# GEOS-ESM/QuickChem

Hardware: AMD Instinct MI355X
Metric: OH gridcells/sec (XGBoost predict), C360 L72 batch (higher is better)
Workload: dtype f32

## Files before the change

quickchem_amd/capi.py:

```python
from __future__ import annotations

import ctypes as C
import os
from typing import Optional, Sequence

import numpy as np

_HERE = os.path.dirname(os.path.abspath(__file__))
LIB_PATH = os.path.join(_HERE, "lib", "libohxgb.so")
RING_ROUNDS_DEFAULT = 64
RING_ROUNDS_NO_GRID = 16
RING_ROUNDS_PERMUTED = 4
VISITS_BLOCK_ROWS = 256
VISITS_LDS_BLOCKS_PER_CU = 1
VISITS_GLOBAL_BLOCKS_PER_CU = 4

ABI_SYMBOLS = [
    "XGBGetLastError", "XGDMatrixCreateFromMat", "XGDMatrixFree", "XGDMatrixNumRow", "XGDMatrixNumCol",
    "XGDMatrixSaveBinary", "XGDMatrixCreateFromFile", "XGBoosterCreate", "XGBoosterFree", "XGBoosterLoadModel",
    "XGBoosterSaveModel", "XGBoosterLoadModelFromBuffer", "XGBoosterPredict", "XGBoosterSetParam",
    "OHXDeviceCount", "OHXDMatrixCreateFromDevice", "OHXDMatrixSetGrid", "OHXDMatrixGetGrid", "OHXDMatrixInferGrid", "OHXBoosterPredictDevice", "OHXBoosterCheck",
    "OHXBoosterPredictContribs", "OHXBoosterPredictContribsDevice",
    "OHXBoosterPredictInteractions", "OHXBoosterPredictInteractionsDevice",
    "OHXBoosterPredictContribsFields", "OHXBoosterPredictContribsFieldsDevice",
    "OHXBoosterCountVisits", "OHXBoosterCountVisitsDevice", "OHXBoosterGetVisitCounts", "OHXBoosterResetVisitCounts",
    "OHXBoosterRefreshCover", "OHXBoosterRefitLeaves", "OHXBoosterRefitLeavesDevice",
    "OHXBoosterBoostTrees", "OHXBoosterBoostTreesDevice", "OHXBoosterBoostTreesEval", "OHXBoosterBoostTreesEvalDevice",
    "OHXBoosterBoostTreesWeighted", "OHXBoosterBoostTreesWeightedDevice",
    "OHXBoosterBoostTreesSampled", "OHXBoosterBoostTreesSampledDevice",
    "OHXBoosterBoostTreesDeep", "OHXBoosterBoostTreesDeepDevice",
    "OHXBoosterBoostTreesDeepSampled", "OHXBoosterBoostTreesDeepSampledDevice",
    "OHXQuantileCuts", "OHXDMatrixQuantileCuts",
    "OHXSelectCells", "OHXSelectCellsDevice", "OHXGatherCells", "OHXGatherCellsDevice",
    "OHXScatterCells", "OHXScatterCellsDevice",
    "OHXBoosterPredictFields", "OHXBoosterPredictFieldsDevice", "OHXBoosterRun1", "OHXBoosterRun1Device", "OHXOHPostProcess", "OHXOHPostProcessDevice",
    "OHXJulianDay", "OHXSolarGeometry", "OHXSolarGeometryDevice", "OHXBoosterGetInfo", "OHXBoosterGetNumGroups", "OHXBoosterGetNumCategoricalSplits", "OHXBoosterKernelSymbol", "OHXBoosterKernelSymbolRows",
    "OHXBoosterRingReruns", "OHXBoosterCopyEngineChoice", "OHXUnregisterHost", "OHXReleaseScratch",
    "OHXCommGetUniqueId", "OHXCommInitRank", "OHXCommFree", "OHXCommInfo", "OHXShardRows", "OHXAllGatherOH",
]
REFERENCE_BOUND_SYMBOLS = [
    "XGBoosterLoadModel", "XGBoosterSaveModel", "XGDMatrixSaveBinary", "XGDMatrixFree", "XGDMatrixCreateFromFile",
    "XGBoosterPredict", "XGBoosterCreate", "XGDMatrixCreateFromMat", "XGDMatrixNumRow", "XGDMatrixNumCol",
    "XGBoosterFree",
# ... 1008 lines not shown
```

quickchem_amd/csrc/capi.cpp:

```cpp
#include <hip/hip_runtime_api.h>

#include <algorithm>
#include <cmath>
#include <cstdio>
#include <cstdlib>
#include <cstring>
#include <fstream>
#include <map>
#include <memory>
#include <atomic>
#include <chrono>
#include <mutex>
#include <unordered_map>
#include <sstream>
#include <string>
#include <unordered_set>
#include <vector>

#include "../../include/ohxgb.h"
#include "categorical.hpp"
#include "cells.hpp"
#include "contribs.hpp"
#include "flatten.hpp"
#include "forest.hpp"
// ... 812 lines not shown
  b.dev = use_device(b.device_pref);
  const Forest& flat = b.flat();
  b.placement = place_forest(flat, b.layout);
  b.packed_ok = packed_format_fits(flat, b.placement);
  b.d_roots.upload(b.placement.roots);
  if (b.num_cat != 0) {
    CatForest cf = emit_cat(flat, b.placement);
    b.cat_word_count = cf.words.size();
    b.cat_inline_sets = cf.inline_sets;
    b.cat_word_sets = cf.word_sets;
    if (cf.words.empty()) cf.words.push_back(0u);
    b.d_cat_nodes.upload(cf.nodes);
    b.d_cat_words.upload(cf.words);
    b.d_cat_orig.upload(cf.orig_id);
  } else if (wants_super(b.kernel_name)) {
    SuperForest sf;
    b.super_ok = emit_super(flat, &sf, b.layout.super_pack) && sf.nodes.size() * sizeof(SuperNode) < 0xFFFFFFF0ull;
    if (b.super_ok) {
      b.super_slots = sf.nodes.size();
      b.super_gathers[0] = count_super_gathers(sf, 0);
      b.super_gathers[1] = count_super_gathers(sf, 1);
      b.super_gathers[2] = count_super_gathers(sf, 2);
      b.super_mean_steps = mean_super_steps(sf);
      b.d_super.upload(sf.nodes);
      if (((uintptr_t)b.d_super.p & 127u) != 0) throw OhxError("internal error: the super-node array is not 128-byte aligned");
      b.d_super_heads.upload(sf.heads);
    }
  }
  if (b.num_cat == 0 && b.packed_ok && !(b.super_ok && wants_super(b.kernel_name))) {
    std::vector<PackedNode> packed = emit_packed(flat, b.placement, nullptr);
    b.d_packed.upload(packed);
  }
  if (b.num_cat == 0 && pick_kernel(b) == KernelKind::Wide) ensure_wide(b);
  b.d_flags.ensure(3);
  {
    LibStreams& ls = lib_streams(b.dev.ordinal);
    b.s_exec = ls.exec;
    b.s_copy = ls.copy;
  }
  HIP_CHECK(hipMemsetAsync(b.d_flags.p, 0, 3 * sizeof(uint32_t), b.s_exec));
  HIP_CHECK(hipStreamSynchronize(b.s_exec));
  b.ring_reruns_seen = 0;
  ensure_train_stream(b);
  b.uploaded = true;
}

void ensure_train_stream(BoosterObj& b) {
  b.tune.train = nullptr;
  if (b.tune.overlap_group < 2) return;
  if (!b.train.side) {
    HIP_CHECK(hipStreamCreateWithFlags(&b.train.side, hipStreamNonBlocking));
    HIP_CHECK(hipEventCreateWithFlags(&b.train.fork, hipEventDisableTiming));
    HIP_CHECK(hipEventCreateWithFlags(&b.train.join, hipEventDisableTiming));
  }
  b.tune.train = &b.train;
}

DeviceForest device_forest(const BoosterObj& b) {
  DeviceForest d;
  d.packed = b.d_packed.p;
  d.wide = b.d_wide.p;
  d.roots = b.d_roots.p;
  d.super = b.d_super.p;
  d.super_heads = b.d_super_heads.p;
  d.packed_bytes = (uint32_t)(b.d_packed.n * sizeof(PackedNode));
  d.super_bytes = (uint32_t)(b.d_super.n * sizeof(SuperNode));
  d.num_trees = (uint32_t)b.forest.trees.size();
  d.num_feature = b.forest.num_feature;
  d.base_score = b.margin_base;
  d.tree_tops = (b.super_ok && use_tree_tops(b.tune, b.super_mean_steps)) ? 1u : 0u;
  return d;
}

// ... 3833 lines not shown
```

quickchem_amd/csrc/kernels.hip:

```cpp
#include <hip/hip_runtime.h>

#include <atomic>

#include <cstdint>

#include "kernels.hpp"
#include "walk_device.hpp"

namespace ohx {

namespace {

constexpr int kBlock = 256;
constexpr int kWavesPerBlock = kBlock / kWave;

typedef const __attribute__((address_space(3))) char* lds_cptr;
typedef const __attribute__((address_space(3))) u32x4* lds_u32x4_ptr;
typedef __attribute__((address_space(3))) uint32_t* lds_u32_ptr;
typedef __attribute__((address_space(3))) void* lds_void_ptr;


__device__ __forceinline__ uint64_t launch_row(const PredictArgs& a, uint64_t tile_id, int lane, bool* valid,
                                               uint64_t perm_slots = ~0ull) {
  if (a.perm != nullptr) {
// ... 624 lines not shown
        const bool lane_nan = stage_rows<true>(tile, a.rows, row, valid, a.ncol, fr.num_feature, a.missing,
                                               missing_is_nan, a.flags);
        float* leaves = a.leaf_buf + ((size_t)(tile_id - a.tile_begin) * ntree - a.tree_begin) * kWave + lane;
        (void)walk_tile<FMT, CHAINS, TOPS>(fr, heads, t0, t1, tile, __any(lane_nan), first, nfirst, leaves);
      }
      return;
    }
  }
  uint64_t slots = ~0ull, tile_end = a.tile_end;
  if (a.perm_count != nullptr) {
    const uint32_t filled = *a.perm_count;
    slots = filled < a.perm_slots ? filled : a.perm_slots;
    const uint64_t need = (slots + kWave - 1) / kWave;
    tile_end = need < tile_end ? need : tile_end;
  }
  for (uint64_t tile_id = a.tile_begin + wave_id; tile_id < tile_end; tile_id += nwaves) {
    bool valid;
    const uint64_t row = launch_row(a, tile_id, lane, &valid, slots);
    if (!__any(valid)) continue;
    const bool lane_nan = stage_rows<true>(tile, a.rows, row, valid, a.ncol, fr.num_feature, a.missing,
                                           missing_is_nan, a.flags);
    const bool wave_nan = __any(lane_nan);
    const float acc = walk_tile<FMT, CHAINS, TOPS>(fr, heads, a.tree_begin, a.tree_end, tile, wave_nan, first, nfirst);
    if (valid) __builtin_nontemporal_store(acc, out + row);
  }
}

constexpr int kRingChains = 4;
constexpr int kRingWaves = 16;
constexpr int kRingBlock = kRingWaves * kWave;
constexpr uint32_t kRingSteps = 4;
constexpr uint32_t kRingSlots = 176;
constexpr uint32_t kRingBuffers = 4;
constexpr uint32_t kRingTreeBytes = kRingSlots * 16u;
constexpr uint32_t kRingBufBytes = kRingChains * kRingTreeBytes;
constexpr uint32_t kRingDmaLoads = kRingChains * kRingSlots / kWave;
static_assert(kRingChains * kRingSlots % kWave == 0, "a group is whole wave loads");
#ifndef OHX_EXP_RING_SPIN
#define OHX_EXP_RING_SPIN (1u << 21)
#endif
constexpr uint32_t kRingSpinLimit = OHX_EXP_RING_SPIN;
constexpr size_t kRingLdsBytes = (size_t)kRingWaves * 27 * kWave * sizeof(float) + (size_t)kRingBuffers * kRingBufBytes +
                                 (size_t)(kRingWaves + 4) * sizeof(uint32_t);
static_assert(kRingLdsBytes <= 160 * 1024, "LDS of a block");

__device__ __forceinline__ uint32_t ring_load(lds_u32_ptr p) {
  return __hip_atomic_load(p, __ATOMIC_RELAXED, __HIP_MEMORY_SCOPE_WORKGROUP);
}
__device__ __forceinline__ void ring_store(lds_u32_ptr p, uint32_t v) {
  __hip_atomic_store(p, v, __ATOMIC_RELAXED, __HIP_MEMORY_SCOPE_WORKGROUP);
}
__device__ __forceinline__ void ring_order() { asm volatile("s_waitcnt lgkmcnt(0)" ::: "memory"); }

__device__ __forceinline__ void dma_to_lds_b128(u32x4 desc, uint32_t off, uint32_t lds_addr) {
#if defined(__gfx950__)
  uint32_t keep;
  const uint32_t m0_value = (uint32_t)__builtin_amdgcn_readfirstlane((int)lds_addr);
  asm volatile(
      "s_mov_b32 %0, m0\n\ts_mov_b32 m0, %3\n\ts_nop 0\n\tbuffer_load_dwordx4 %1, %2, 0 offen lds\n\ts_mov_b32 m0, %0"
      : "=&s"(keep)
      : "v"(off), "s"(desc), "s"(m0_value)
      : "memory");
#else
  (void)desc; (void)off; (void)lds_addr;
  __builtin_trap();
#endif
}

struct TopRing {
  lds_cptr ring;
  uint32_t ring_addr;
  lds_u32_ptr progress, filled, claim, abort;
  u32x4 desc;
  __amdgpu_buffer_rsrc_t forest;
  const SuperTreeHead* heads;
  uint32_t t0, t1, ngroups;
  uint32_t total;
  uint32_t g;
  bool gave_up;
};

__device__ __forceinline__ void ring_stage(const TopRing& rg, uint32_t first_tree, uint32_t buf, int lane) {
  uint32_t base[kRingChains];
#pragma unroll
  for (int c = 0; c < kRingChains; ++c) base[c] = rg.heads[(first_tree + c < rg.t1) ? first_tree + c : rg.t1 - 1].base;
#pragma unroll
  for (uint32_t q = 0; q < kRingDmaLoads; ++q) {
    const uint32_t L = q * kWave + (uint32_t)lane;
    uint32_t b = base[0], rec = L;
#pragma unroll
    for (int k = 1; k < kRingChains; ++k)
      if (L >= (uint32_t)k * kRingSlots) b = base[k], rec = L - (uint32_t)k * kRingSlots;
    dma_to_lds_b128(rg.desc, (b + rec) << 4, rg.ring_addr + buf * kRingBufBytes + q * 1024u);
  }
}

__device__ __forceinline__ void ring_begin(TopRing& rg, char* ring, const DeviceForest& fr, const SuperTreeHead* heads,
                                           uint32_t t0, uint32_t t1, uint32_t rounds) {
  const int lane = threadIdx.x & (kWave - 1);
  rg.ring = (lds_cptr)ring;
  rg.ring_addr = (uint32_t)(uintptr_t)(lds_void_ptr)ring;
  rg.progress = (lds_u32_ptr)(ring + (size_t)kRingBuffers * kRingBufBytes);
  rg.filled = rg.progress + kRingWaves;
  rg.claim = rg.progress + kRingWaves + 1;
  rg.abort = rg.progress + kRingWaves + 2;
  const uint64_t addr = reinterpret_cast<uint64_t>(fr.super);
  rg.desc.x = (uint32_t)__builtin_amdgcn_readfirstlane((int)(uint32_t)addr);
  rg.desc.y = (uint32_t)__builtin_amdgcn_readfirstlane((int)((uint32_t)(addr >> 32) & 0xFFFFu));
  rg.desc.z = (uint32_t)__builtin_amdgcn_readfirstlane((int)fr.super_bytes);
  rg.desc.w = 0x00020000u;
  rg.forest = make_rsrc(fr.super, fr.super_bytes);
  rg.heads = heads;
  rg.t0 = t0;
  rg.t1 = t1;
  rg.ngroups = (t1 - t0 + kRingChains - 1) / kRingChains;
  rg.total = rounds * rg.ngroups;
  rg.g = 0;
  rg.gave_up = false;
  if (threadIdx.x < kWave) {
    ring_stage(rg, t0, 0u, lane);
    asm volatile("s_waitcnt vmcnt(0)" ::: "memory");
  }
  if (threadIdx.x < (uint32_t)kRingWaves) ring_store(rg.progress + threadIdx.x, 0u);
  if (threadIdx.x == 0) {
    ring_store(rg.filled, 1u);
    ring_store(rg.claim, 1u);
    ring_store(rg.abort, 0u);
  }
  __syncthreads();
}

template <bool HAS_MISSING>
__device__ __forceinline__ float ring_walk_group(const SuperTreeHead (&h)[kRingChains], uint32_t ntrees_here,
                                                 __amdgpu_buffer_rsrc_t forest, const float* __restrict__ tile,
                                                 lds_cptr tops, float acc, lds_u32_ptr publish_to,
                                                 uint32_t publish_value, bool ahead) {
  constexpr int CHAINS = kRingChains;
  const char* tile_b = reinterpret_cast<const char*>(tile);
  __builtin_amdgcn_s_setprio(1);
  u32x4 s[CHAINS];
  uint32_t rel[CHAINS], leafb[CHAINS];
  float xr[CHAINS];
#pragma unroll
  for (int c = 0; c < CHAINS; ++c) xr[c] = tile[(h[c].root_meta & 31u) * kWave];
#pragma unroll
  for (int c = 0; c < CHAINS; ++c) {
    bool l = xr[c] < h[c].root_thr;
    if (HAS_MISSING) l = go_left_or_default(xr[c], h[c].root_thr, (h[c].root_meta & 32u) != 0u);
    rel[c] = 4u + (((h[c].root_meta & 0x100u) && !l) ? 1u : 0u);
    leafb[c] = 0u;
  }
  uint32_t nsteps = h[0].steps;
#pragma unroll
  for (int c = 1; c < CHAINS; ++c) nsteps = h[c].steps > nsteps ? h[c].steps : nsteps;
  nsteps = nsteps < kRingSteps ? kRingSteps : nsteps;
#pragma unroll
  for (int c = 0; c < CHAINS; ++c) s[c] = *(lds_u32x4_ptr)(tops + (uint32_t)c * kRingTreeBytes + (rel[c] << 4));
#pragma unroll
  for (uint32_t step = 1; step < kRingSteps; ++step) {
    if (step == 2 && !ahead) __builtin_amdgcn_s_setprio(2);
    super_step<CHAINS, HAS_MISSING, false>(s, rel, leafb, tile_b);
#pragma unroll
    for (int c = 0; c < CHAINS; ++c) s[c] = *(lds_u32x4_ptr)(tops + (uint32_t)c * kRingTreeBytes + (rel[c] << 4));
  }
  if (publish_to != nullptr) {
    asm volatile("s_waitcnt vmcnt(0)" ::: "memory");
    if ((threadIdx.x & (kWave - 1)) == 0) ring_store(publish_to, publish_value);
  }
  if (ahead) __builtin_amdgcn_s_setprio(2);
  else __builtin_amdgcn_s_setprio(3);
  uint32_t base[CHAINS];
#pragma unroll
  for (int c = 0; c < CHAINS; ++c) base[c] = h[c].base;
  for (uint32_t step = kRingSteps; step < nsteps; ++step)
    super_step_by_chain<CHAINS, HAS_MISSING>(s, rel, leafb, tile_b, [&](int c, uint32_t record) -> u32x4 {
      return __builtin_amdgcn_raw_buffer_load_b128(forest, (int)((base[c] + record) << 4), 0, 0);
    });
  super_step<CHAINS, HAS_MISSING, true>(s, rel, leafb, tile_b);
  __builtin_amdgcn_s_setprio(1);
#pragma unroll
  for (int c = 0; c < CHAINS; ++c)
    if ((uint32_t)c < ntrees_here) acc += __uint_as_float(leafb[c]);
  return acc;
}

__device__ __forceinline__ bool ring_aborted(const TopRing& rg) {
  return __builtin_amdgcn_readfirstlane((int)ring_load(rg.abort)) != 0;
}

__device__ __forceinline__ void ring_give_up(TopRing& rg, int lane) {
  rg.gave_up = true;
  if (lane == 0) ring_store(rg.abort, 1u);
}

__device__ __forceinline__ float ring_walk_tile(TopRing& rg, float acc, const float* __restrict__ tile, bool live,
                                                bool wave_nan, int lane, int wave) {
  if (rg.gave_up) return acc;
  for (uint32_t p = 0; p < rg.ngroups; ++p, ++rg.g) {
    const uint32_t g = rg.g;
    const uint32_t t = rg.t0 + p * kRingChains;
    uint32_t won = 0;
    uint32_t filled_now = 0;
    if (lane == 0) {
      uint32_t expected = g + 1u;
      const bool may = g + 1u < rg.total && !rg.gave_up;
      filled_now = ring_load(rg.filled);
      if (may) won = __hip_atomic_compare_exchange_strong(rg.claim, &expected, g + 2u, __ATOMIC_RELAXED, __ATOMIC_RELAXED,
                                                          __HIP_MEMORY_SCOPE_WORKGROUP) ? 1u : 0u;
    }
    won = (uint32_t)__builtin_amdgcn_readfirstlane((int)won);
    filled_now = (uint32_t)__builtin_amdgcn_readfirstlane((int)filled_now);
    if (won || filled_now < g + 1u) __builtin_amdgcn_s_setprio(0);
    if (won) {
      const uint32_t need = g + 2u > kRingBuffers ? g + 2u - kRingBuffers : 0u;
      uint32_t spin = 0;
      while (!__all(lane >= kRingWaves || ring_load(rg.progress + (lane < kRingWaves ? lane : 0)) >= need)) {
        __builtin_amdgcn_s_sleep(2);
        if (++spin > kRingSpinLimit || ring_aborted(rg)) { ring_give_up(rg, lane); break; }
      }
      ring_order();
      if (!rg.gave_up) ring_stage(rg, (p + 1 == rg.ngroups) ? rg.t0 : t + kRingChains, (g + 1u) % kRingBuffers, lane);
    }
    if (filled_now < g + 1u && !rg.gave_up) {
      uint32_t spin = 0;
      while ((uint32_t)__builtin_amdgcn_readfirstlane((int)ring_load(rg.filled)) < g + 1u) {
        __builtin_amdgcn_s_sleep(1);
        if (++spin > kRingSpinLimit || ring_aborted(rg)) { ring_give_up(rg, lane); break; }
      }
    }
    ring_order();
    const lds_u32_ptr pub = won ? rg.filled : (lds_u32_ptr) nullptr;
    if (live && !rg.gave_up) {
      SuperTreeHead h[kRingChains];
#pragma unroll
      for (int c = 0; c < kRingChains; ++c) h[c] = rg.heads[(t + c < rg.t1) ? t + c : rg.t1 - 1];
      const uint32_t here = rg.t1 - t < (uint32_t)kRingChains ? rg.t1 - t : (uint32_t)kRingChains;
      const lds_cptr buf = rg.ring + (g % kRingBuffers) * kRingBufBytes;
      acc = wave_nan ? ring_walk_group<true>(h, here, rg.forest, tile, buf, acc, pub, g + 2u, won != 0u)
                     : ring_walk_group<false>(h, here, rg.forest, tile, buf, acc, pub, g + 2u, won != 0u);
    } else if (won) {
      asm volatile("s_waitcnt vmcnt(0)" ::: "memory");
      if (lane == 0 && !rg.gave_up) ring_store(rg.filled, g + 2u);
    }
    ring_order();
    if (lane == 0) ring_store(rg.progress + wave, g + 1u);
  }
  __builtin_amdgcn_s_setprio(0);
  return acc;
}

__global__ __launch_bounds__(kRingBlock) __attribute__((amdgpu_waves_per_eu(4))) void predict_rows_ring_kernel(
    DeviceForest fr, PredictArgs a, const SuperTreeHead* __restrict__ heads, float* __restrict__ out) {
  extern __shared__ float lds[];
  const int lane = threadIdx.x & (kWave - 1);
  const int wave = threadIdx.x / kWave;
  float* tile = lds + (size_t)wave * 27 * kWave + lane;
  float* tile_base = tile - lane;
  const bool missing_is_nan = a.missing != a.missing;
  uint32_t block = blockIdx.x;
  if (a.xcd_remap && (gridDim.x & 7u) == 0u) block = (blockIdx.x & 7u) * (gridDim.x >> 3) + (blockIdx.x >> 3);
  const uint64_t wave_id = (uint64_t)block * kRingWaves + wave;
  const uint64_t nwaves = (uint64_t)gridDim.x * kRingWaves;
  const uint64_t first_tile = a.tile_begin + (uint64_t)block * kRingWaves;
  if (first_tile >= a.tile_end) return;
  const uint32_t rounds = (uint32_t)((a.tile_end - first_tile + nwaves - 1) / nwaves);
  TopRing rg;
  ring_begin(rg, reinterpret_cast<char*>(lds + (size_t)kRingWaves * 27 * kWave), fr, heads, a.tree_begin, a.tree_end, rounds);
  uint64_t tile_id = a.tile_begin + wave_id;
  Row27 regs;
  bool valid = false, together = false;
  uint64_t row = 0;
  if (tile_id < a.tile_end) {
    row = launch_row(a, tile_id, lane, &valid);
    together = a.run_log >= 2u && !__any(valid && (row == 0 || row + 1 == a.nrow));
    if (together) load_pieces(regs, a, row, lane);
    else load_row27(regs, a.rows, valid ? row : 0);
  }
  for (uint32_t r = 0; r < rounds; ++r) {
    const bool live = tile_id < a.tile_end && __any(valid);
    const bool lane_nan = !live ? false
                          : together ? store_pieces(tile_base, regs, a, __ballot(valid), lane, missing_is_nan)
                                     : store_row27(tile, regs, valid, a.missing, missing_is_nan, a.flags);
    const uint64_t next = tile_id + nwaves;
    const uint64_t this_row = row;
    const bool this_valid = valid;
    if (next < a.tile_end) {
      row = launch_row(a, next, lane, &valid);
      together = a.run_log >= 2u && !__any(valid && (row == 0 || row + 1 == a.nrow));
      if (together) load_pieces(regs, a, row, lane);
      else load_row27(regs, a.rows, valid ? row : 0);
    } else {
      valid = false;
    }
    bool wave_nan = __any(lane_nan);
    bool keep = this_valid;
    __builtin_amdgcn_fence(__ATOMIC_RELEASE, "wavefront");
    __builtin_amdgcn_wave_barrier();
    __builtin_amdgcn_fence(__ATOMIC_ACQUIRE, "wavefront");
    if (wave_nan && a.defer_count != nullptr && a.defer_cap == 0u) {
      if ((tile_id & 7u) == 0u) {
        const uint32_t n = 8u * (uint32_t)__popcll(__ballot(lane_nan));
        if (lane == 0) atomicAdd(a.defer_count, n);
      }
    } else if (wave_nan && a.defer_count != nullptr) {
      bool mine = false;
#pragma unroll
      for (int f = 0; f < 27; ++f) {
        const float x = tile[f * kWave];
        mine |= (x != x);
      }
      const bool leaves = mine && this_valid;
      const uint64_t who = __ballot(leaves);
      const uint32_t n = (uint32_t)__popcll(who);
      uint32_t at = 0;
      if (lane == 0) at = atomicAdd(a.defer_count, n);
      at = (uint32_t)__builtin_amdgcn_readfirstlane((int)at);
      if (at + n <= a.defer_cap) {
        if (leaves) a.defer_list[at + (uint32_t)__popcll(who & ((1ull << lane) - 1ull))] = (uint32_t)this_row;
        keep = this_valid && !mine;
        wave_nan = false;
      }
    }
    const float acc = ring_walk_tile(rg, fr.base_score, tile, live, wave_nan, lane, wave);
    if (live && keep && !rg.gave_up) __builtin_nontemporal_store(acc, out + this_row);
    tile_id = next;
  }
  if (rg.gave_up && a.flags && lane == 0) atomicExch(a.flags + 2, a.train_id);
}

__global__ __launch_bounds__(kRingBlock) __attribute__((amdgpu_waves_per_eu(4))) void predict_fields_ring_kernel(
    DeviceForest fr, FieldsArgs a, const SuperTreeHead* __restrict__ heads, float* __restrict__ out,
    float* __restrict__ margin_out) {
  extern __shared__ float lds[];
  const int lane = threadIdx.x & (kWave - 1);
  const int wave = threadIdx.x / kWave;
  float* tile = lds + (size_t)wave * 27 * kWave + lane;
  const bool missing_is_nan = a.missing != a.missing;
  const uint64_t plane = (uint64_t)a.im * (uint64_t)a.jm;
  const uint64_t nrow = plane * (uint64_t)(a.k2 - a.k1 + 1);
  const uint64_t slab = level_floats(a, plane) * (uint64_t)(a.k1 - a.src_k0);
  const uint64_t slab_out = level_floats(a, plane) * (uint64_t)(a.k1 - a.out_k0);
  uint32_t block = blockIdx.x;
  if (a.xcd_remap && (gridDim.x & 7u) == 0u) block = (blockIdx.x & 7u) * (gridDim.x >> 3) + (blockIdx.x >> 3);
  const uint64_t wave_id = (uint64_t)block * kRingWaves + wave;
  const uint64_t nwaves = (uint64_t)gridDim.x * kRingWaves;
  const uint64_t first_tile = a.tile_begin + (uint64_t)block * kRingWaves;
  if (first_tile >= a.tile_end) return;
  const uint32_t rounds = (uint32_t)((a.tile_end - first_tile + nwaves - 1) / nwaves);
  TopRing rg;
  ring_begin(rg, reinterpret_cast<char*>(lds + (size_t)kRingWaves * 27 * kWave), fr, heads, a.tree_begin, a.tree_end, rounds);
  uint64_t tile_id = a.tile_begin + wave_id;
  for (uint32_t r = 0; r < rounds; ++r, tile_id += nwaves) {
    bool valid = false;
    uint64_t m = 0;
    if (tile_id < a.tile_end) m = tile_row(a.shape, tile_id, lane, nrow, &valid);
    const bool live = __any(valid);
    const CellAt at = cell_at(a, plane, valid ? m : 0);
    const bool lane_nan = live && fill_tile_fields(a, tile, 27u, at.at3, at.at2, slab, valid, missing_is_nan);
    bool wave_nan = __any(lane_nan);
    bool keep = valid;
    if (wave_nan && a.defer_count != nullptr && a.defer_cap == 0u) {
      if ((tile_id & 7u) == 0u) {
        const uint32_t n = 8u * (uint32_t)__popcll(__ballot(lane_nan && valid));
        if (lane == 0) atomicAdd(a.defer_count, n);
      }
    } else if (wave_nan && a.defer_count != nullptr) {
      const bool leaves = lane_nan && valid;
      const uint64_t who = __ballot(leaves);
      const uint32_t n = (uint32_t)__popcll(who);
      uint32_t at = 0;
      if (lane == 0) at = atomicAdd(a.defer_count, n);
      at = (uint32_t)__builtin_amdgcn_readfirstlane((int)at);
      if (at + n <= a.defer_cap) {
        if (leaves) a.defer_list[at + (uint32_t)__popcll(who & ((1ull << lane) - 1ull))] = (uint32_t)m;
        keep = valid && !lane_nan;
        wave_nan = false;
      }
    }
    const float acc = ring_walk_tile(rg, fr.base_score, tile, live, wave_nan, lane, wave);
    if (keep && !rg.gave_up) store_oh(a, out, margin_out, slab_out, m, at.at3, acc);
  }
  if (rg.gave_up && a.flags && lane == 0) atomicExch(a.flags + 2, a.train_id);
}

__global__ __launch_bounds__(kBlock) void combine_leaves_kernel(PredictArgs a, float base_score, float* __restrict__ out) {
  const int lane = threadIdx.x & (kWave - 1);
  const uint64_t ntiles = a.tile_end - a.tile_begin, nwaves = (uint64_t)gridDim.x * kWavesPerBlock;
  const uint32_t ntree = a.tree_end - a.tree_begin;
  for (uint64_t w = (uint64_t)blockIdx.x * kWavesPerBlock + threadIdx.x / kWave; w < ntiles; w += nwaves) {
    bool valid;
    const uint64_t row = launch_row(a, a.tile_begin + w, lane, &valid);
    if (!__any(valid)) continue;
    const float* leaves = a.leaf_buf + (size_t)w * ntree * kWave + lane;
    float acc = base_score;
#pragma unroll 4
    for (uint32_t t = 0; t < ntree; ++t) acc += leaves[(size_t)t * kWave];
    if (valid) out[row] = acc;
  }
}

template <bool PRED_LEAF>
__global__ __launch_bounds__(kBlock) void predict_rows_direct_kernel(DeviceForest fr, PredictArgs a) {
  const uint4* nodes = reinterpret_cast<const uint4*>(fr.wide);
  const bool missing_is_nan = a.missing != a.missing;
  const bool missing_is_inf = is_inf(a.missing);
  const uint32_t ntree = a.tree_end - a.tree_begin;
  const uint64_t stride = (uint64_t)gridDim.x * blockDim.x;
  for (uint64_t row = (uint64_t)blockIdx.x * blockDim.x + threadIdx.x; row < a.nrow; row += stride) {
    const float* x = a.rows + row * (uint64_t)a.ncol;
    float acc = fr.base_score;
    bool any_inf = false;
    for (uint32_t t = a.tree_begin; t < a.tree_end; ++t) {
      uint4 nd = nodes[fr.roots[t]];
// ... 538 lines not shown
        hipError_t e = hipEventRecord(tr->fork, main);
        if (e != hipSuccess) return e;
        e = hipStreamWaitEvent(tr->side, tr->fork, 0);
        if (e != hipSuccess) return e;
        side_open = true;
      }
      *out = tr->side;
    }
    return hipSuccess;
  }
};


using RowsKernel = void (*)(DeviceForest, PredictArgs, const SuperTreeHead*, float*);
using FieldsKernel = void (*)(DeviceForest, FieldsArgs, const SuperTreeHead*, float*, float*);

void launch_walk(RowsKernel kernel, uint64_t grid, unsigned threads, size_t lds, hipStream_t stream, const DeviceForest& fr,
                 const PredictArgs& a) {
  hipLaunchKernelGGL(kernel, dim3((unsigned)grid), dim3(threads), lds, stream, fr, a, fr.super_heads, a.out);
}
void launch_walk(FieldsKernel kernel, uint64_t grid, unsigned threads, size_t lds, hipStream_t stream, const DeviceForest& fr,
                 const FieldsArgs& a) {
  hipLaunchKernelGGL(kernel, dim3((unsigned)grid), dim3(threads), lds, stream, fr, a, fr.super_heads, a.out, a.margin_out);
}
void launch_combine(unsigned grid, hipStream_t stream, const DeviceForest& fr, const PredictArgs& a) {
  hipLaunchKernelGGL(combine_leaves_kernel, dim3(grid), dim3(kBlock), 0, stream, a, fr.base_score, a.out);
}
void launch_combine(unsigned grid, hipStream_t stream, const DeviceForest& fr, const FieldsArgs& a) {
  hipLaunchKernelGGL(combine_leaves_fields_kernel, dim3(grid), dim3(kBlock), 0, stream, a, fr.base_score, a.out, a.margin_out);
}

template <class K, class Args>
hipError_t launch_train(K kernel, unsigned threads, size_t lds, uint64_t grid, uint64_t ntiles, uint64_t per_launch,
                        hipStream_t stream, const LaunchTuning& tune, const DeviceForest& fr, Args a) {
  const uint64_t waves = threads / kWave;
  TrainCursor train(stream, tune);
  for (uint64_t t0 = 0; t0 < ntiles; t0 += per_launch) {
    a.tile_begin = t0;
    a.tile_end = t0 + per_launch < ntiles ? t0 + per_launch : ntiles;
    const uint64_t blocks = (a.tile_end - a.tile_begin + waves - 1) / waves;
    hipStream_t s;
    hipError_t e = train.next(&s);
    if (e != hipSuccess) return e;
    launch_walk(kernel, blocks < grid ? blocks : grid, threads, lds, s, fr, a);
  }
  return train.meet();
}

template <class K, class Args>
hipError_t launch_ring_rerun(K again, size_t lds, const DeviceForest& fr, Args b, uint64_t ntiles, int num_cus, hipStream_t stream) {
  hipError_t e = raise_lds_limit(again, lds);
  if (e != hipSuccess) return e;
  b.only_if_train = b.train_id;
  b.defer_list = nullptr;
  b.defer_count = nullptr;
  b.defer_cap = 0;
  b.tile_begin = 0;
  b.tile_end = ntiles;
  launch_walk(again, tile_grid(again, lds, ntiles, num_cus), kBlock, lds, stream, fr, b);
  return hipSuccess;
}

template <class K, class Args>
hipError_t launch_deferred(K kernel, size_t lds, const DeviceForest& fr, Args a, int num_cus, hipStream_t stream) {
  hipError_t e = raise_lds_limit(kernel, lds);
  if (e != hipSuccess) return e;
  a.perm = a.defer_list;
  a.perm_count = a.defer_count;
  a.perm_slots = a.defer_cap;
  a.defer_list = nullptr;
  a.defer_count = nullptr;
  a.tile_begin = 0;
  a.tile_end = ((uint64_t)a.defer_cap + kWave - 1) / kWave;
  launch_walk(kernel, tile_grid(kernel, lds, a.tile_end, num_cus), kBlock, lds, stream, fr, a);
  return hipSuccess;
}
// ... 192 lines not shown
  return nullptr;
}

FieldsKernel fields_ring_later_kernel() { return predict_fields_kernel<2, 2, true>; }


template <class K, class Args>
hipError_t launch_plan(const WalkPlan& p, K first, K rerun, K second, const DeviceForest& fr, Args a, uint64_t nrow, int num_cus,
                       hipStream_t stream, const LaunchTuning& tune) {
  if (first == nullptr || rerun == nullptr || second == nullptr) return hipErrorInvalidValue;
  a.shape = p.shape;
  a.xcd_remap = tune.xcd_remap;
  const uint64_t ntiles = p.shape.ntiles(nrow);
  if (p.defer) {
    a.defer_cap = p.defer_cap;
    a.defer_count = tune.defer_buf;
    a.defer_list = tune.defer_buf + 1;
    hipError_t e = hipMemsetAsync(a.defer_count, 0, sizeof(uint32_t), stream);
    if (e == hipSuccess && p.listing) e = hipMemsetAsync(a.defer_list, 0xFF, (size_t)a.defer_cap * sizeof(uint32_t), stream);
    if (e != hipSuccess) return e;
  }
  if (p.how == WalkPlan::Split) {
    hipError_t e = launch_split(first, p.lds, fr, a, ntiles, num_cus, stream, tune, p.split);
    return e != hipSuccess ? e : hipGetLastError();
  }
  hipError_t e = raise_lds_limit(first, p.lds);
  if (e != hipSuccess) return e;
  set_runs(a, p.runs);
  const bool ring = p.how == WalkPlan::Ring;
  const unsigned threads = ring ? kRingBlock : kBlock;
  const uint64_t waves = threads / kWave;
  uint64_t grid = (ntiles + waves - 1) / waves;
  if (ring) {
    if (grid > p.cus) grid = p.cus;
    a.train_id = next_train_id();
  } else {
    grid = (uint64_t)tile_grid(first, p.lds, ntiles, num_cus);
  }
  e = launch_train(first, threads, p.lds, grid, ntiles, p.rounds <= 0 ? ntiles : grid * waves * (uint64_t)p.rounds, stream, tune, fr, a);
  if (e == hipSuccess && ring && a.flags != nullptr) e = launch_ring_rerun(rerun, p.lds_tile, fr, a, ntiles, num_cus, stream);
  if (e == hipSuccess && p.listing) {
    set_runs(a, CoopRuns());
    a.shape = TileShape();
    e = launch_deferred(second, p.lds_tile, fr, a, num_cus, stream);
  }
  return e != hipSuccess ? e : hipGetLastError();
}

std::string rows_tile_symbol(const WalkPlan& p, bool pf) {
  return "predict_rows_tile_kernel<" + std::to_string(p.fmt) + "," + std::to_string(p.chains) + (pf ? ",true," : ",false,") +
         (p.tops ? "true>" : "false>");
}

}

const char* kernel_kind_name(KernelKind k) {
  switch (k) {
    case KernelKind::Wide: return "wide";
    case KernelKind::Packed1: return "packed1";
    case KernelKind::Packed2: return "packed2";
    case KernelKind::Packed4: return "packed4";
    case KernelKind::Super1: return "super1";
    case KernelKind::Super2: return "super2";
    case KernelKind::Super3: return "super3";
    case KernelKind::Super4: return "super4";
    case KernelKind::Ring: return "ring";
  }
  return "?";
}

hipError_t launch_predict(KernelKind kind, const DeviceForest& fr, const PredictArgs& a, int num_cus, hipStream_t stream,
                          const LaunchTuning& tune) {
// ... 180 lines not shown
```

quickchem_amd/csrc/kernels.hpp:

```cpp
#pragma once
#include <hip/hip_runtime_api.h>

#include <cstdint>
#include <string>

#include "flatten.hpp"

namespace ohx {

enum : uint32_t {
  kFlagInfInput = 1u,
};

constexpr uint32_t kFirstStepTrees = 128;

struct DeviceForest {
  const PackedNode* packed = nullptr;
  const WideNode* wide = nullptr;
  const uint32_t* roots = nullptr;
  const int32_t* packed_orig_id = nullptr;
  const SuperNode* super = nullptr;
  const SuperTreeHead* super_heads = nullptr;
  uint32_t num_trees = 0;
  uint32_t num_feature = 0;
// ... 37 lines not shown
    k_first = (uint32_t)(row0 / plane);
    nk = (uint32_t)((row0 + nrow - 1) / plane) - k_first + 1;
    nbi = (im + (1u << li) - 1) >> li;
    nbj = (jm + (1u << lj) - 1) >> lj;
    nbk = (nk + (1u << lk) - 1) >> lk;
  }
  void set_grid_auto(uint32_t im_, uint32_t jm_, uint64_t row0_, uint64_t nrow_) {
    static const uint32_t cand3[3][3] = {{2, 2, 2}, {3, 2, 1}, {3, 3, 0}};
    static const uint32_t cand1[3][3] = {{3, 0, 3}, {4, 0, 2}, {5, 0, 1}};
    static const double speed3[3] = {1.0, 0.994, 0.98}, speed1[3] = {1.0, 0.99, 0.94};
    const uint32_t (*cand)[3] = jm_ == 1 ? cand1 : cand3;
    const double* speed = jm_ == 1 ? speed1 : speed3;
    double best = -1.0;
    int pick = 0;
    for (int q = 0; q < 3; ++q) {
      set_grid(im_, jm_, row0_, nrow_, cand[q][0], cand[q][1], cand[q][2]);
      const double score = fill() * speed[q];
      if (score > best) best = score, pick = q;
    }
    set_grid(im_, jm_, row0_, nrow_, cand[pick][0], cand[pick][1], cand[pick][2]);
  }
};

struct PredictArgs {
  const float* rows = nullptr;
  uint64_t nrow = 0;
  uint32_t ncol = 0;
  float missing = 0.0f;
  uint32_t tree_begin = 0, tree_end = 0;
  float* out = nullptr;
  bool pred_leaf = false;
  uint32_t* flags = nullptr;
  uint32_t train_id = 0, only_if_train = 0;
  uint64_t tile_begin = 0;
  uint64_t tile_end = 0;
  int xcd_remap = 1;
  const uint32_t* perm = nullptr;
  const uint32_t* perm_count = nullptr;
  uint32_t perm_slots = 0;
  uint32_t* defer_list = nullptr;
  uint32_t* defer_count = nullptr;
  uint32_t defer_cap = 0;
  float* leaf_buf = nullptr;
  uint32_t tree_split = 1;
  uint32_t run_log = 0, run_lo_bits = 0;
  TileShape shape;
};

struct TrainStreams {
  hipStream_t side = nullptr;
  hipEvent_t fork = nullptr, join = nullptr;
};

constexpr int kRingRoundsNoGrid = 16;
constexpr int kRingRoundsPermuted = 4;

struct LaunchTuning {
  int launches_per_residency = 2;
  int xcd_remap = 1;
  int overlap_group = 0;
  const TrainStreams* train = nullptr;
  int tree_tops = -1;
  int prefetch = 1;
  int coop_rows = 1;
  int lds_pad = 0;
  int ring_rounds = 64;
  int run1_pieces = 0;
  int reserve_cus = 0;
  int tree_split = -1;
  float* leaf_buf = nullptr;
  size_t leaf_words = 0;
  int defer_missing = -1;
  int defer_count_only = 0;
  uint32_t* defer_buf = nullptr;
  size_t defer_words = 0;
  int cluster = -1;
  int cluster_trees = 2, cluster_steps = 7, cluster_zorder = 0;
  int grid_im = 0, grid_jm = 0;
  uint64_t grid_row0 = 0;
  int brick_li = -1, brick_lj = -1, brick_lk = -1;
  int brick_k_fastest = 1;
};

struct FieldsArgs {
  const float* field[32];
  uint32_t is2d_mask = 0;
  uint32_t pl_feature = 1;
  uint32_t nfield = 0;
  int im = 0, jm = 0, km = 0, k1 = 0, k2 = 0;
  uint64_t level_stride = 0;
  int src_k0 = 0;
  int out_k0 = 0;
  float missing = 0.0f;
  uint32_t tree_begin = 0, tree_end = 0;
  int apply_pow10 = 1;
  float scale = 1.0f;
  float* out = nullptr;
  float* margin_out = nullptr;
  uint32_t* flags = nullptr;
  uint32_t train_id = 0, only_if_train = 0;
  uint64_t tile_begin = 0, tile_end = 0;
  int xcd_remap = 1;
  TileShape shape;
  uint32_t* defer_list = nullptr;
  uint32_t* defer_count = nullptr;
  uint32_t defer_cap = 0;
  const uint32_t* perm = nullptr;
  const uint32_t* perm_count = nullptr;
  uint32_t perm_slots = 0;
  float* leaf_buf = nullptr;
  uint32_t tree_split = 1;
};

struct PrepArgs {
  int im = 0, jm = 0, km = 0;
  uint64_t col0 = 0, ncols = 0;
  int beside_a_walk = 0;
  const float *ple_bst = nullptr, *zle_bst = nullptr, *tauclw = nullptr, *taucli = nullptr;
  const float* sca[7] = {};
  const float *gmito3 = nullptr, *gmitto3 = nullptr;
  float *pl_bst = nullptr, *tauclwdn = nullptr, *tauclidn = nullptr, *taucliup = nullptr, *tauclwup = nullptr;
  float *aodup = nullptr, *aoddn = nullptr, *strato3 = nullptr;
};

struct SlabArgs {
  int im = 0, jm = 0, km = 0;
  int dynamic_k_range = 1;
  float tropp_min = 4000.0f;
  const float *ple_mod = nullptr, *tropp = nullptr;
  int32_t* result = nullptr;
};

struct PostArgs {
// ... 121 lines not shown
```

Before: 2.454 billion.

## Replace static ring-kernel round striding with atomic dynamic work claiming

The persistent ring kernels no longer give each block a fixed stride of tiles. Blocks now claim their next round of tiles from a global atomic counter, and the claimed round is staged ahead through a small LDS slot array so the prefetch pipeline knows where to go next. The default ring_rounds becomes 0, so the whole grid runs in a single persistent launch instead of many relaunches. This targets load imbalance and relaunch overhead at the tail, at the cost of extra atomics, a memset per launch, and more complex synchronisation inside the ring.

```diff
diff --git a/quickchem_amd/capi.py b/quickchem_amd/capi.py
--- a/quickchem_amd/capi.py
+++ b/quickchem_amd/capi.py
@@ -8,7 +8,7 @@
 
 _HERE = os.path.dirname(os.path.abspath(__file__))
 LIB_PATH = os.path.join(_HERE, "lib", "libohxgb.so")
-RING_ROUNDS_DEFAULT = 64
+RING_ROUNDS_DEFAULT = 0
 RING_ROUNDS_NO_GRID = 16
 RING_ROUNDS_PERMUTED = 4
 VISITS_BLOCK_ROWS = 256
diff --git a/quickchem_amd/csrc/capi.cpp b/quickchem_amd/csrc/capi.cpp
--- a/quickchem_amd/csrc/capi.cpp
+++ b/quickchem_amd/csrc/capi.cpp
@@ -868,13 +868,13 @@
     b.d_packed.upload(packed);
   }
   if (b.num_cat == 0 && pick_kernel(b) == KernelKind::Wide) ensure_wide(b);
-  b.d_flags.ensure(3);
+  b.d_flags.ensure(kFlagWords);
   {
     LibStreams& ls = lib_streams(b.dev.ordinal);
     b.s_exec = ls.exec;
     b.s_copy = ls.copy;
   }
-  HIP_CHECK(hipMemsetAsync(b.d_flags.p, 0, 3 * sizeof(uint32_t), b.s_exec));
+  HIP_CHECK(hipMemsetAsync(b.d_flags.p, 0, kFlagWords * sizeof(uint32_t), b.s_exec));
   HIP_CHECK(hipStreamSynchronize(b.s_exec));
   b.ring_reruns_seen = 0;
   ensure_train_stream(b);
diff --git a/quickchem_amd/csrc/kernels.hip b/quickchem_amd/csrc/kernels.hip
--- a/quickchem_amd/csrc/kernels.hip
+++ b/quickchem_amd/csrc/kernels.hip
@@ -680,6 +680,8 @@
 constexpr uint32_t kRingSteps = 4;
 constexpr uint32_t kRingSlots = 176;
 constexpr uint32_t kRingBuffers = 4;
+constexpr uint32_t kRingRoundSlots = 8;
+constexpr uint32_t kNoRound = 0xFFFFFFFFu;
 constexpr uint32_t kRingTreeBytes = kRingSlots * 16u;
 constexpr uint32_t kRingBufBytes = kRingChains * kRingTreeBytes;
 constexpr uint32_t kRingDmaLoads = kRingChains * kRingSlots / kWave;
@@ -689,7 +691,7 @@
 #endif
 constexpr uint32_t kRingSpinLimit = OHX_EXP_RING_SPIN;
 constexpr size_t kRingLdsBytes = (size_t)kRingWaves * 27 * kWave * sizeof(float) + (size_t)kRingBuffers * kRingBufBytes +
-                                 (size_t)(kRingWaves + 4) * sizeof(uint32_t);
+                                 (size_t)(kRingWaves + 4 + kRingRoundSlots) * sizeof(uint32_t);
 static_assert(kRingLdsBytes <= 160 * 1024, "LDS of a block");
 
 __device__ __forceinline__ uint32_t ring_load(lds_u32_ptr p) {
@@ -719,15 +721,24 @@
   lds_cptr ring;
   uint32_t ring_addr;
   lds_u32_ptr progress, filled, claim, abort;
+  lds_u32_ptr rounds;
+  uint32_t* claims;
+  uint32_t block;
   u32x4 desc;
   __amdgpu_buffer_rsrc_t forest;
   const SuperTreeHead* heads;
   uint32_t t0, t1, ngroups;
-  uint32_t total;
+  uint32_t nrounds;
+  uint32_t ord, next;
   uint32_t g;
   bool gave_up;
 };
 
+__device__ __forceinline__ uint32_t ring_round_of(uint32_t nrounds, uint32_t claimed) {
+  const uint32_t round = gridDim.x + claimed;
+  return (round >= gridDim.x && round < nrounds) ? round : kNoRound;
+}
+
 __device__ __forceinline__ void ring_stage(const TopRing& rg, uint32_t first_tree, uint32_t buf, int lane) {
   uint32_t base[kRingChains];
 #pragma unroll
@@ -743,8 +754,12 @@
   }
 }
 
+__device__ __forceinline__ uint32_t ring_claim(uint32_t* claims, uint32_t block, uint32_t j, uint32_t n) {
+  return claims != nullptr ? atomicAdd(claims, n) : block + (j - 1u) * gridDim.x;
+}
+
 __device__ __forceinline__ void ring_begin(TopRing& rg, char* ring, const DeviceForest& fr, const SuperTreeHead* heads,
-                                           uint32_t t0, uint32_t t1, uint32_t rounds) {
+                                           uint32_t t0, uint32_t t1, uint32_t nrounds, uint32_t* claims, uint32_t block) {
   const int lane = threadIdx.x & (kWave - 1);
   rg.ring = (lds_cptr)ring;
   rg.ring_addr = (uint32_t)(uintptr_t)(lds_void_ptr)ring;
@@ -752,6 +767,12 @@
   rg.filled = rg.progress + kRingWaves;
   rg.claim = rg.progress + kRingWaves + 1;
   rg.abort = rg.progress + kRingWaves + 2;
+  rg.rounds = rg.progress + kRingWaves + 4;
+  rg.claims = claims;
+  rg.block = block;
+  rg.nrounds = nrounds;
+  rg.ord = 0;
+  rg.next = kNoRound;
   const uint64_t addr = reinterpret_cast<uint64_t>(fr.super);
   rg.desc.x = (uint32_t)__builtin_amdgcn_readfirstlane((int)(uint32_t)addr);
   rg.desc.y = (uint32_t)__builtin_amdgcn_readfirstlane((int)((uint32_t)(addr >> 32) & 0xFFFFu));
@@ -762,12 +783,19 @@
   rg.t0 = t0;
   rg.t1 = t1;
   rg.ngroups = (t1 - t0 + kRingChains - 1) / kRingChains;
-  rg.total = rounds * rg.ngroups;
   rg.g = 0;
   rg.gave_up = false;
   if (threadIdx.x < kWave) {
+    const uint32_t ahead = rg.ngroups == 1u ? 2u : 1u;
+    uint32_t claimed = 0;
+    if (lane == 0) claimed = ring_claim(claims, block, 1u, ahead);
     ring_stage(rg, t0, 0u, lane);
     asm volatile("s_waitcnt vmcnt(0)" ::: "memory");
+    if (lane < (int)kRingRoundSlots) ring_store(rg.rounds + lane, kNoRound);
+    if (lane == 0) {
+      ring_store(rg.rounds + 1, ring_round_of(nrounds, claimed));
+      if (ahead == 2u) ring_store(rg.rounds + 2, ring_round_of(nrounds, claimed + (claims != nullptr ? 1u : gridDim.x)));
+    }
   }
   if (threadIdx.x < (uint32_t)kRingWaves) ring_store(rg.progress + threadIdx.x, 0u);
   if (threadIdx.x == 0) {
@@ -782,7 +810,8 @@
 __device__ __forceinline__ float ring_walk_group(const SuperTreeHead (&h)[kRingChains], uint32_t ntrees_here,
                                                  __amdgpu_buffer_rsrc_t forest, const float* __restrict__ tile,
                                                  lds_cptr tops, float acc, lds_u32_ptr publish_to,
-                                                 uint32_t publish_value, bool ahead) {
+                                                 uint32_t publish_value, bool ahead, lds_u32_ptr round_to,
+                                                 uint32_t claimed, uint32_t nrounds) {
   constexpr int CHAINS = kRingChains;
   const char* tile_b = reinterpret_cast<const char*>(tile);
   __builtin_amdgcn_s_setprio(1);
@@ -813,7 +842,11 @@
   }
   if (publish_to != nullptr) {
     asm volatile("s_waitcnt vmcnt(0)" ::: "memory");
-    if ((threadIdx.x & (kWave - 1)) == 0) ring_store(publish_to, publish_value);
+    if ((threadIdx.x & (kWave - 1)) == 0) {
+      if (round_to != nullptr) ring_store(round_to, ring_round_of(nrounds, claimed));
+      asm volatile("" ::: "memory");
+      ring_store(publish_to, publish_value);
+    }
   }
   if (ahead) __builtin_amdgcn_s_setprio(2);
   else __builtin_amdgcn_s_setprio(3);
@@ -851,7 +884,7 @@
     uint32_t filled_now = 0;
     if (lane == 0) {
       uint32_t expected = g + 1u;
-      const bool may = g + 1u < rg.total && !rg.gave_up;
+      const bool may = (p + 1u < rg.ngroups || rg.next != kNoRound) && !rg.gave_up;
       filled_now = ring_load(rg.filled);
       if (may) won = __hip_atomic_compare_exchange_strong(rg.claim, &expected, g + 2u, __ATOMIC_RELAXED, __ATOMIC_RELAXED,
                                                           __HIP_MEMORY_SCOPE_WORKGROUP) ? 1u : 0u;
@@ -878,23 +911,44 @@
     }
     ring_order();
     const lds_u32_ptr pub = won ? rg.filled : (lds_u32_ptr) nullptr;
+    lds_u32_ptr round_to = (lds_u32_ptr) nullptr;
+    uint32_t claimed = 0;
+    if (won && !rg.gave_up && (p + 2u == rg.ngroups || rg.ngroups == 1u)) {
+      const uint32_t far = rg.ngroups == 1u ? 3u : 2u;
+      uint32_t before = rg.next;
+      if (far == 3u) before = (uint32_t)__builtin_amdgcn_readfirstlane((int)ring_load(rg.rounds + ((rg.ord + 2u) % kRingRoundSlots)));
+      if (before != kNoRound) {
+        if (lane == 0) claimed = ring_claim(rg.claims, rg.block, rg.ord + far, 1u);
+        round_to = rg.rounds + ((rg.ord + far) % kRingRoundSlots);
+      }
+    }
     if (live && !rg.gave_up) {
       SuperTreeHead h[kRingChains];
 #pragma unroll
       for (int c = 0; c < kRingChains; ++c) h[c] = rg.heads[(t + c < rg.t1) ? t + c : rg.t1 - 1];
       const uint32_t here = rg.t1 - t < (uint32_t)kRingChains ? rg.t1 - t : (uint32_t)kRingChains;
       const lds_cptr buf = rg.ring + (g % kRingBuffers) * kRingBufBytes;
-      acc = wave_nan ? ring_walk_group<true>(h, here, rg.forest, tile, buf, acc, pub, g + 2u, won != 0u)
-                     : ring_walk_group<false>(h, here, rg.forest, tile, buf, acc, pub, g + 2u, won != 0u);
+      acc = wave_nan ? ring_walk_group<true>(h, here, rg.forest, tile, buf, acc, pub, g + 2u, won != 0u, round_to, claimed, rg.nrounds)
+                     : ring_walk_group<false>(h, here, rg.forest, tile, buf, acc, pub, g + 2u, won != 0u, round_to, claimed, rg.nrounds);
     } else if (won) {
       asm volatile("s_waitcnt vmcnt(0)" ::: "memory");
-      if (lane == 0 && !rg.gave_up) ring_store(rg.filled, g + 2u);
+      if (lane == 0 && !rg.gave_up) {
+        if (round_to != nullptr) ring_store(round_to, ring_round_of(rg.nrounds, claimed));
+        asm volatile("" ::: "memory");
+        ring_store(rg.filled, g + 2u);
+      }
     }
     ring_order();
     if (lane == 0) ring_store(rg.progress + wave, g + 1u);
   }
   __builtin_amdgcn_s_setprio(0);
+  ++rg.ord;
   return acc;
+}
+
+__device__ __forceinline__ uint32_t ring_next_round(TopRing& rg) {
+  rg.next = (uint32_t)__builtin_amdgcn_readfirstlane((int)ring_load(rg.rounds + ((rg.ord + 1u) % kRingRoundSlots)));
+  return rg.next;
 }
 
 __global__ __launch_bounds__(kRingBlock) __attribute__((amdgpu_waves_per_eu(4))) void predict_rows_ring_kernel(
@@ -907,14 +961,12 @@
   const bool missing_is_nan = a.missing != a.missing;
   uint32_t block = blockIdx.x;
   if (a.xcd_remap && (gridDim.x & 7u) == 0u) block = (blockIdx.x & 7u) * (gridDim.x >> 3) + (blockIdx.x >> 3);
-  const uint64_t wave_id = (uint64_t)block * kRingWaves + wave;
-  const uint64_t nwaves = (uint64_t)gridDim.x * kRingWaves;
-  const uint64_t first_tile = a.tile_begin + (uint64_t)block * kRingWaves;
-  if (first_tile >= a.tile_end) return;
-  const uint32_t rounds = (uint32_t)((a.tile_end - first_tile + nwaves - 1) / nwaves);
+  const uint32_t nrounds = (uint32_t)((a.tile_end - a.tile_begin + kRingWaves - 1) / kRingWaves);
+  if (block >= nrounds) return;
   TopRing rg;
-  ring_begin(rg, reinterpret_cast<char*>(lds + (size_t)kRingWaves * 27 * kWave), fr, heads, a.tree_begin, a.tree_end, rounds);
-  uint64_t tile_id = a.tile_begin + wave_id;
+  ring_begin(rg, reinterpret_cast<char*>(lds + (size_t)kRingWaves * 27 * kWave), fr, heads, a.tree_begin, a.tree_end, nrounds,
+             a.ring_claims, block);
+  uint64_t tile_id = a.tile_begin + (uint64_t)block * kRingWaves + wave;
   Row27 regs;
   bool valid = false, together = false;
   uint64_t row = 0;
@@ -924,12 +976,13 @@
     if (together) load_pieces(regs, a, row, lane);
     else load_row27(regs, a.rows, valid ? row : 0);
   }
-  for (uint32_t r = 0; r < rounds; ++r) {
+  for (;;) {
     const bool live = tile_id < a.tile_end && __any(valid);
     const bool lane_nan = !live ? false
                           : together ? store_pieces(tile_base, regs, a, __ballot(valid), lane, missing_is_nan)
                                      : store_row27(tile, regs, valid, a.missing, missing_is_nan, a.flags);
-    const uint64_t next = tile_id + nwaves;
+    const uint32_t next_round = ring_next_round(rg);
+    const uint64_t next = next_round != kNoRound ? a.tile_begin + (uint64_t)next_round * kRingWaves + wave : a.tile_end;
     const uint64_t this_row = row;
     const bool this_valid = valid;
     if (next < a.tile_end) {
@@ -971,6 +1024,7 @@
     }
     const float acc = ring_walk_tile(rg, fr.base_score, tile, live, wave_nan, lane, wave);
     if (live && keep && !rg.gave_up) __builtin_nontemporal_store(acc, out + this_row);
+    if (next_round == kNoRound || rg.gave_up) break;
     tile_id = next;
   }
   if (rg.gave_up && a.flags && lane == 0) atomicExch(a.flags + 2, a.train_id);
@@ -990,15 +1044,14 @@
   const uint64_t slab_out = level_floats(a, plane) * (uint64_t)(a.k1 - a.out_k0);
   uint32_t block = blockIdx.x;
   if (a.xcd_remap && (gridDim.x & 7u) == 0u) block = (blockIdx.x & 7u) * (gridDim.x >> 3) + (blockIdx.x >> 3);
-  const uint64_t wave_id = (uint64_t)block * kRingWaves + wave;
-  const uint64_t nwaves = (uint64_t)gridDim.x * kRingWaves;
-  const uint64_t first_tile = a.tile_begin + (uint64_t)block * kRingWaves;
-  if (first_tile >= a.tile_end) return;
-  const uint32_t rounds = (uint32_t)((a.tile_end - first_tile + nwaves - 1) / nwaves);
+  const uint32_t nrounds = (uint32_t)((a.tile_end - a.tile_begin + kRingWaves - 1) / kRingWaves);
+  if (block >= nrounds) return;
   TopRing rg;
-  ring_begin(rg, reinterpret_cast<char*>(lds + (size_t)kRingWaves * 27 * kWave), fr, heads, a.tree_begin, a.tree_end, rounds);
-  uint64_t tile_id = a.tile_begin + wave_id;
-  for (uint32_t r = 0; r < rounds; ++r, tile_id += nwaves) {
+  ring_begin(rg, reinterpret_cast<char*>(lds + (size_t)kRingWaves * 27 * kWave), fr, heads, a.tree_begin, a.tree_end, nrounds,
+             a.ring_claims, block);
+  uint64_t tile_id = a.tile_begin + (uint64_t)block * kRingWaves + wave;
+  for (;;) {
+    const uint32_t next_round = ring_next_round(rg);
     bool valid = false;
     uint64_t m = 0;
     if (tile_id < a.tile_end) m = tile_row(a.shape, tile_id, lane, nrow, &valid);
@@ -1027,6 +1080,8 @@
     }
     const float acc = ring_walk_tile(rg, fr.base_score, tile, live, wave_nan, lane, wave);
     if (keep && !rg.gave_up) store_oh(a, out, margin_out, slab_out, m, at.at3, acc);
+    if (next_round == kNoRound || rg.gave_up) break;
+    tile_id = a.tile_begin + (uint64_t)next_round * kRingWaves + wave;
   }
   if (rg.gave_up && a.flags && lane == 0) atomicExch(a.flags + 2, a.train_id);
 }
@@ -1631,7 +1686,7 @@
 
 template <class K, class Args>
 hipError_t launch_train(K kernel, unsigned threads, size_t lds, uint64_t grid, uint64_t ntiles, uint64_t per_launch,
-                        hipStream_t stream, const LaunchTuning& tune, const DeviceForest& fr, Args a) {
+                        hipStream_t stream, const LaunchTuning& tune, const DeviceForest& fr, Args a, uint32_t* claims = nullptr) {
   const uint64_t waves = threads / kWave;
   TrainCursor train(stream, tune);
   for (uint64_t t0 = 0; t0 < ntiles; t0 += per_launch) {
@@ -1641,6 +1696,11 @@
     hipStream_t s;
     hipError_t e = train.next(&s);
     if (e != hipSuccess) return e;
+    if (claims != nullptr) {
+      a.ring_claims = claims + (s == stream ? 0 : 1);
+      e = hipMemsetAsync(a.ring_claims, 0, sizeof(uint32_t), s);
+      if (e != hipSuccess) return e;
+    }
     launch_walk(kernel, blocks < grid ? blocks : grid, threads, lds, s, fr, a);
   }
   return train.meet();
@@ -1899,12 +1959,16 @@
   const uint64_t waves = threads / kWave;
   uint64_t grid = (ntiles + waves - 1) / waves;
   if (ring) {
+    if (a.flags == nullptr) return hipErrorInvalidValue;
     if (grid > p.cus) grid = p.cus;
     a.train_id = next_train_id();
   } else {
     grid = (uint64_t)tile_grid(first, p.lds, ntiles, num_cus);
   }
-  e = launch_train(first, threads, p.lds, grid, ntiles, p.rounds <= 0 ? ntiles : grid * waves * (uint64_t)p.rounds, stream, tune, fr, a);
+  uint64_t per_launch = p.rounds <= 0 ? ntiles : grid * waves * (uint64_t)p.rounds;
+  if (ring && per_launch > (uint64_t)0x7FFFFFFFu * waves) per_launch = (uint64_t)0x7FFFFFFFu * waves;
+  e = launch_train(first, threads, p.lds, grid, ntiles, per_launch, stream, tune, fr, a,
+                   ring && p.shape.im != 0 ? a.flags + 3 : nullptr);
   if (e == hipSuccess && ring && a.flags != nullptr) e = launch_ring_rerun(rerun, p.lds_tile, fr, a, ntiles, num_cus, stream);
   if (e == hipSuccess && p.listing) {
     set_runs(a, CoopRuns());
diff --git a/quickchem_amd/csrc/kernels.hpp b/quickchem_amd/csrc/kernels.hpp
--- a/quickchem_amd/csrc/kernels.hpp
+++ b/quickchem_amd/csrc/kernels.hpp
@@ -93,6 +93,7 @@
   bool pred_leaf = false;
   uint32_t* flags = nullptr;
   uint32_t train_id = 0, only_if_train = 0;
+  uint32_t* ring_claims = nullptr;
   uint64_t tile_begin = 0;
   uint64_t tile_end = 0;
   int xcd_remap = 1;
@@ -115,6 +116,7 @@
 
 constexpr int kRingRoundsNoGrid = 16;
 constexpr int kRingRoundsPermuted = 4;
+constexpr int kFlagWords = 5;
 
 struct LaunchTuning {
   int launches_per_residency = 2;
@@ -125,7 +127,7 @@
   int prefetch = 1;
   int coop_rows = 1;
   int lds_pad = 0;
-  int ring_rounds = 64;
+  int ring_rounds = 0;
   int run1_pieces = 0;
   int reserve_cus = 0;
   int tree_split = -1;
@@ -160,6 +162,7 @@
   float* margin_out = nullptr;
   uint32_t* flags = nullptr;
   uint32_t train_id = 0, only_if_train = 0;
+  uint32_t* ring_claims = nullptr;
   uint64_t tile_begin = 0, tile_end = 0;
   int xcd_remap = 1;
   TileShape shape;
```

After: 2.467 billion (median of 6 runs). About the same (+0.6%).
